# sus0pid/hsig-picotls

Measured on AMD Instinct MI355X. Metric: GiB/s AES-128-GCM seal+open, device-resident, 16KiB records, 1/2/4/8 GPU, higher is better.
Workload: dtype u8; 1 GPU; AES-128-GCM, 1M x 16 KiB TLS records, single key, per GPU (BASELINE configs[1]); records_per_gpu=1048576, record_bytes=16384, aad_bytes=5, keys=1, key_bits=128, lanes_per_record=4, record_align=128, parallelism=records sharded by range over 1 GPU(s), no collective

## Files before the change

hsig-picotls_amd/csrc/batch_kernel.h:

```cpp
#ifndef PTLS_HIP_BATCH_KERNEL_H
#define PTLS_HIP_BATCH_KERNEL_H

#include <hip/hip_runtime.h>
#include <type_traits>
#include "internal.h"

namespace ptls_hip {

constexpr uint32_t LDS_GMAIN = 0;
constexpr uint32_t LDS_AES = 65536;
constexpr uint32_t LDS_GTREE = 131072;
constexpr uint32_t LDS_TREE_STRIDE = 8192;
constexpr int TREE_TABLES = 3;
__host__ __device__ constexpr uint32_t lds_bytes(int log2g)
{
    return (void)log2g, LDS_GTREE + TREE_TABLES * LDS_TREE_STRIDE;
}

constexpr int SETPRIO = 1;
constexpr int PURE_BLOCKS = 2;
#ifndef DEAL_MUTANT
#define DEAL_MUTANT 0
#endif
#ifndef KS_STAMPS
#define KS_STAMPS 0
#endif
constexpr int QRING = 32;
constexpr uint32_t Q_END = 0xffffffffu;

struct V4 {
    uint32_t w0, w1, w2, w3;
};

__device__ __forceinline__ V4 v4xor(V4 a, V4 b)
{
    return V4{a.w0 ^ b.w0, a.w1 ^ b.w1, a.w2 ^ b.w2, a.w3 ^ b.w3};
}

__device__ __forceinline__ uint32_t xor3(uint32_t a, uint32_t b, uint32_t c)
{
    return __builtin_amdgcn_bitop3_b32(a, b, c, 0x96);
}

__device__ __forceinline__ V4 v4xor3(V4 a, V4 b, V4 c)
{
    return V4{xor3(a.w0, b.w0, c.w0), xor3(a.w1, b.w1, c.w1), xor3(a.w2, b.w2, c.w2), xor3(a.w3, b.w3, c.w3)};
}

__device__ __forceinline__ uint32_t bswap32(uint32_t x)
{
    return __builtin_bswap32(x);
}

__device__ __forceinline__ uint32_t lds32(const uint8_t *lds, uint32_t addr)
{
    return *reinterpret_cast<const uint32_t *>(lds + addr);
}

__device__ __forceinline__ V4 lds128(const uint8_t *lds, uint32_t addr)
{
    const uint4 v = *reinterpret_cast<const uint4 *>(lds + addr);
    return V4{v.x, v.y, v.z, v.w};
}

__device__ __forceinline__ void lds128_store(uint8_t *lds, uint32_t addr, V4 v)
{
    *reinterpret_cast<uint4 *>(lds + addr) = make_uint4(v.w0, v.w1, v.w2, v.w3);
}


template <int K>
__device__ __forceinline__ uint32_t aes_addr(uint32_t x, uint32_t lb)
{
    static_assert(LDS_AES == 65536, "the table base is injected as byte 2 of the address");
    return __builtin_amdgcn_perm(x, lb, 0x0c020000u | ((4u + K) << 8));
}

__device__ __forceinline__ uint32_t rotl8(uint32_t x)
{
    return __builtin_amdgcn_alignbit(x, x, 24);
}

__device__ __forceinline__ uint32_t aes_col(const uint8_t *lds, uint32_t lb, uint32_t x0, uint32_t x1, uint32_t x2, uint32_t x3,
                                            uint32_t k)
{
    const uint32_t a0 = lds32(lds, aes_addr<0>(x0, lb));
    const uint32_t a1 = lds32(lds, aes_addr<1>(x1, lb));
    const uint32_t a2 = lds32(lds, 128 + aes_addr<2>(x2, lb));
    const uint32_t a3 = lds32(lds, 128 + aes_addr<3>(x3, lb));
    return xor3(a0, a2, rotl8(a1 ^ a3)) ^ k;
}

__device__ __forceinline__ uint32_t aes_col_last(const uint8_t *lds, uint32_t lb, uint32_t x0, uint32_t x1, uint32_t x2,
                                                 uint32_t x3, uint32_t k)
{
    const uint32_t u0 = lds32(lds, 128 + aes_addr<0>(x0, lb));
    const uint32_t u1 = lds32(lds, aes_addr<1>(x1, lb));
    const uint32_t u2 = lds32(lds, aes_addr<2>(x2, lb));
    const uint32_t u3 = lds32(lds, 128 + aes_addr<3>(x3, lb));
    const uint32_t lo = __builtin_amdgcn_perm(u1, u0, 0x0c0c0500u);
    const uint32_t hi = __builtin_amdgcn_perm(u3, u2, 0x07020c0cu);
    return xor3(lo, hi, k);
}

template <int ROUNDS>
__device__ __forceinline__ V4 aes_encrypt(const uint8_t *lds, uint32_t lb, const uint32_t *__restrict__ rk, V4 s)
{
    s.w0 ^= rk[0];
    s.w1 ^= rk[1];
    s.w2 ^= rk[2];
    s.w3 ^= rk[3];
#pragma unroll
    for (int r = 1; r < ROUNDS; ++r) {
        const uint32_t t0 = aes_col(lds, lb, s.w0, s.w1, s.w2, s.w3, rk[4 * r + 0]);
        const uint32_t t1 = aes_col(lds, lb, s.w1, s.w2, s.w3, s.w0, rk[4 * r + 1]);
        const uint32_t t2 = aes_col(lds, lb, s.w2, s.w3, s.w0, s.w1, rk[4 * r + 2]);
        const uint32_t t3 = aes_col(lds, lb, s.w3, s.w0, s.w1, s.w2, rk[4 * r + 3]);
        s = V4{t0, t1, t2, t3};
    }
    const uint32_t t0 = aes_col_last(lds, lb, s.w0, s.w1, s.w2, s.w3, rk[4 * ROUNDS + 0]);
    const uint32_t t1 = aes_col_last(lds, lb, s.w1, s.w2, s.w3, s.w0, rk[4 * ROUNDS + 1]);
    const uint32_t t2 = aes_col_last(lds, lb, s.w2, s.w3, s.w0, s.w1, rk[4 * ROUNDS + 2]);
    const uint32_t t3 = aes_col_last(lds, lb, s.w3, s.w0, s.w1, s.w2, rk[4 * ROUNDS + 3]);
    return V4{t0, t1, t2, t3};
}

template <int K>
__device__ __forceinline__ uint32_t lT0(const uint8_t *lds, uint32_t x, uint32_t lb)
{
    return lds32(lds, aes_addr<K>(x, lb));
}
template <int K>
__device__ __forceinline__ uint32_t lT2(const uint8_t *lds, uint32_t x, uint32_t lb)
{
    return lds32(lds, 128 + aes_addr<K>(x, lb));
}

struct CtrConst {
    uint32_t k10, k11;
    uint32_t k20, k21, k22, k23;
    uint32_t r03;
};

__device__ __forceinline__ CtrConst ctr_const(const uint8_t *lds, uint32_t lb, const uint32_t *__restrict__ rk, uint32_t n0,
                                              uint32_t n1, uint32_t n2)
{
    const uint32_t s0 = n0 ^ rk[0], s1 = n1 ^ rk[1], s2 = n2 ^ rk[2], s3 = rk[3];
    CtrConst c;
    c.r03 = rk[3];
    c.k10 = lT0<0>(lds, s0, lb) ^ rotl8(lT0<1>(lds, s1, lb)) ^ lT2<2>(lds, s2, lb) ^ rk[4];
    c.k11 = lT0<0>(lds, s1, lb) ^ rotl8(lT0<1>(lds, s2, lb)) ^ rotl8(lT2<3>(lds, s0, lb)) ^ rk[5];
    const uint32_t t2 = lT0<0>(lds, s2, lb) ^ rotl8(lT0<1>(lds, s3, lb)) ^ lT2<2>(lds, s0, lb) ^ rotl8(lT2<3>(lds, s1, lb)) ^ rk[6];
    const uint32_t t3 = lT0<0>(lds, s3, lb) ^ rotl8(lT0<1>(lds, s0, lb)) ^ lT2<2>(lds, s1, lb) ^ rotl8(lT2<3>(lds, s2, lb)) ^ rk[7];
    c.k20 = lT2<2>(lds, t2, lb) ^ rotl8(lT2<3>(lds, t3, lb)) ^ rk[8];
    c.k21 = rotl8(lT0<1>(lds, t2, lb)) ^ lT2<2>(lds, t3, lb) ^ rk[9];
    c.k22 = lT0<0>(lds, t2, lb) ^ rotl8(lT0<1>(lds, t3, lb)) ^ rk[10];
    c.k23 = lT0<0>(lds, t3, lb) ^ rotl8(lT2<3>(lds, t2, lb)) ^ rk[11];
    return c;
}

struct RoundLoads {
    uint32_t L[16];
};

__device__ __forceinline__ void round_issue(const uint8_t *lds, uint32_t lb, const V4 &s, RoundLoads &r)
{
    const uint32_t w[4] = {s.w0, s.w1, s.w2, s.w3};
#pragma unroll
    for (int c = 0; c < 4; ++c) {
        r.L[4 * c + 0] = lds32(lds, aes_addr<0>(w[c], lb));
        r.L[4 * c + 1] = lds32(lds, aes_addr<1>(w[(c + 1) & 3], lb));
        r.L[4 * c + 2] = lds32(lds, 128 + aes_addr<2>(w[(c + 2) & 3], lb));
        r.L[4 * c + 3] = lds32(lds, 128 + aes_addr<3>(w[(c + 3) & 3], lb));
    }
}

__device__ __forceinline__ V4 round_finish(const RoundLoads &r, const uint32_t *__restrict__ k)
{
    uint32_t t[4];
#pragma unroll
    for (int c = 0; c < 4; ++c)
        t[c] = xor3(r.L[4 * c + 0], r.L[4 * c + 2], rotl8(r.L[4 * c + 1] ^ r.L[4 * c + 3])) ^ k[c];
    return V4{t[0], t[1], t[2], t[3]};
}

__device__ __forceinline__ void last_issue(const uint8_t *lds, uint32_t lb, const V4 &s, RoundLoads &r)
{
    const uint32_t w[4] = {s.w0, s.w1, s.w2, s.w3};
#pragma unroll
    for (int c = 0; c < 4; ++c) {
        r.L[4 * c + 0] = lds32(lds, 128 + aes_addr<0>(w[c], lb));
        r.L[4 * c + 1] = lds32(lds, aes_addr<1>(w[(c + 1) & 3], lb));
        r.L[4 * c + 2] = lds32(lds, aes_addr<2>(w[(c + 2) & 3], lb));
        r.L[4 * c + 3] = lds32(lds, 128 + aes_addr<3>(w[(c + 3) & 3], lb));
    }
}

__device__ __forceinline__ V4 last_finish(const RoundLoads &r, const uint32_t *__restrict__ k)
{
    uint32_t t[4];
#pragma unroll
    for (int c = 0; c < 4; ++c) {
        const uint32_t lo = __builtin_amdgcn_perm(r.L[4 * c + 1], r.L[4 * c + 0], 0x0c0c0500u);
        const uint32_t hi = __builtin_amdgcn_perm(r.L[4 * c + 3], r.L[4 * c + 2], 0x07020c0cu);
        t[c] = xor3(lo, hi, k[c]);
    }
    return V4{t[0], t[1], t[2], t[3]};
}

template <int ROUNDS, int KP, bool HASH, class GH>
__device__ __forceinline__ void ctr_ghash_skewed(const uint8_t *lds, uint32_t lb, const uint32_t *__restrict__ rk, const CtrConst &cc,
                                                 const uint32_t (&cw)[KP], V4 (&ks)[KP], V4 &y, const V4 (&hx)[KP], const GH &gm)
{
    constexpr int P = GH::PARTS;
    static_assert(P * KP <= KP * ROUNDS, "GHASH parts must fit in the segments");
    V4 s[KP];
    uint32_t t0[KP], t1[KP];
    RoundLoads R[KP];
    uint32_t M[KP][8];
    V4 G[4];
    V4 acc = V4{0, 0, 0, 0}, xr = V4{0, 0, 0, 0};
    constexpr int NSEG = KP * ROUNDS + KP - 1;
#pragma unroll
    for (int seg = 0; seg < NSEG; ++seg) {
        const int gj = seg / P, gq = seg % P;
        const bool gh = HASH && gj < KP;
        __builtin_amdgcn_s_setprio(SETPRIO);
        if (gh) {
            if (gq == 0) {
                xr = gm.prep(y);
                acc = hx[gj];
            }
            switch (gq) {
            case 0: gm.template issue<0>(lds, xr, G); break;
            case 1: gm.template issue<1>(lds, xr, G); break;
            case 2: gm.template issue<2>(lds, xr, G); break;
            case 3: gm.template issue<3 % P>(lds, xr, G); break;
            case 4: gm.template issue<4 % P>(lds, xr, G); break;
            case 5: gm.template issue<5 % P>(lds, xr, G); break;
            case 6: gm.template issue<6 % P>(lds, xr, G); break;
            default: gm.template issue<7 % P>(lds, xr, G); break;
            }
        }
        __builtin_amdgcn_sched_barrier(0);
        if (seg < KP * ROUNDS) {
            const int b = seg % KP, r = seg / KP + 1;
            if (r == 1) {
                const uint32_t x3 = cw[b] ^ cc.r03;
                M[b][0] = lT2<3>(lds, x3, lb);
                M[b][1] = lT2<2>(lds, x3, lb);
            } else if (r == 2) {
                M[b][0] = lT0<0>(lds, t0[b], lb);
                M[b][1] = lT0<1>(lds, t1[b], lb);
                M[b][2] = lT0<0>(lds, t1[b], lb);
                M[b][3] = lT2<3>(lds, t0[b], lb);
                M[b][4] = lT2<2>(lds, t0[b], lb);
                M[b][5] = lT2<3>(lds, t1[b], lb);
                M[b][6] = lT0<1>(lds, t0[b], lb);
                M[b][7] = lT2<2>(lds, t1[b], lb);
            } else if (r < ROUNDS) {
                round_issue(lds, lb, s[b], R[b]);
            } else {
                last_issue(lds, lb, s[b], R[b]);
            }
        }
        __builtin_amdgcn_sched_barrier(0);
        __builtin_amdgcn_s_setprio(0);
        if (seg >= KP - 1) {
            const int fs = seg - (KP - 1);
            const int b = fs % KP, r = fs / KP + 1;
            if (r == 1) {
                t0[b] = cc.k10 ^ rotl8(M[b][0]);
                t1[b] = cc.k11 ^ M[b][1];
            } else if (r == 2) {
                s[b].w0 = xor3(cc.k20, M[b][0], rotl8(M[b][1]));
                s[b].w1 = xor3(cc.k21, M[b][2], rotl8(M[b][3]));
                s[b].w2 = xor3(cc.k22, M[b][4], rotl8(M[b][5]));
                s[b].w3 = xor3(cc.k23, rotl8(M[b][6]), M[b][7]);
            } else if (r < ROUNDS) {
                s[b] = round_finish(R[b], rk + 4 * r);
            } else {
                ks[b] = last_finish(R[b], rk + 4 * r);
            }
        }
        if (gh) {
            acc = v4xor3(acc, G[0], G[1]);
            acc = v4xor3(acc, G[2], G[3]);
            if (gq == P - 1)
                y = acc;
        }
        __builtin_amdgcn_sched_barrier(0);
    }
}

template <int ROUNDS, int K>
__device__ __forceinline__ void aes_encrypt_n(const uint8_t *lds, uint32_t lb, const uint32_t *__restrict__ rk, V4 (&s)[K])
{
#pragma unroll
    for (int b = 0; b < K; ++b) {
        s[b].w0 ^= rk[0];
        s[b].w1 ^= rk[1];
        s[b].w2 ^= rk[2];
        s[b].w3 ^= rk[3];
    }
#pragma unroll
    for (int r = 1; r < ROUNDS; ++r) {
        const uint32_t k0 = rk[4 * r + 0], k1 = rk[4 * r + 1], k2 = rk[4 * r + 2], k3 = rk[4 * r + 3];
        V4 t[K];
#pragma unroll
        for (int b = 0; b < K; ++b) {
            t[b].w0 = aes_col(lds, lb, s[b].w0, s[b].w1, s[b].w2, s[b].w3, k0);
            t[b].w1 = aes_col(lds, lb, s[b].w1, s[b].w2, s[b].w3, s[b].w0, k1);
            t[b].w2 = aes_col(lds, lb, s[b].w2, s[b].w3, s[b].w0, s[b].w1, k2);
            t[b].w3 = aes_col(lds, lb, s[b].w3, s[b].w0, s[b].w1, s[b].w2, k3);
        }
#pragma unroll
        for (int b = 0; b < K; ++b)
            s[b] = t[b];
    }
    const uint32_t k0 = rk[4 * ROUNDS + 0], k1 = rk[4 * ROUNDS + 1], k2 = rk[4 * ROUNDS + 2], k3 = rk[4 * ROUNDS + 3];
    V4 t[K];
#pragma unroll
    for (int b = 0; b < K; ++b) {
        t[b].w0 = aes_col_last(lds, lb, s[b].w0, s[b].w1, s[b].w2, s[b].w3, k0);
        t[b].w1 = aes_col_last(lds, lb, s[b].w1, s[b].w2, s[b].w3, s[b].w0, k1);
        t[b].w2 = aes_col_last(lds, lb, s[b].w2, s[b].w3, s[b].w0, s[b].w1, k2);
        t[b].w3 = aes_col_last(lds, lb, s[b].w3, s[b].w0, s[b].w1, s[b].w2, k3);
    }
#pragma unroll
    for (int b = 0; b < K; ++b)
        s[b] = t[b];
}


struct GhLane {
    uint32_t lb0, lb1, lb2, lb3;
    uint32_t shift;
    bool rot1, rot2;
};

__device__ __forceinline__ GhLane gh_lane_from(uint32_t lane)
{
    GhLane g;
    const uint32_t base = lane * 0x01010101u + 0x03020100u;
    g.lb0 = ((base + 0x00000000u) & 0x0f0f0f0fu) << 4;
    g.lb1 = ((base + 0x04040404u) & 0x0f0f0f0fu) << 4;
    g.lb2 = ((base + 0x08080808u) & 0x0f0f0f0fu) << 4;
    g.lb3 = ((base + 0x0c0c0c0cu) & 0x0f0f0f0fu) << 4;
    g.shift = 8u * (lane & 3);
    g.rot1 = ((lane >> 2) & 1) != 0;
    g.rot2 = ((lane >> 3) & 1) != 0;
    return g;
}

__device__ __forceinline__ GhLane gh_lane_init(int lane)
{
    return gh_lane_from((uint32_t)lane);
}

template <int K>
__device__ __forceinline__ V4 gh_term(const uint8_t *lds, uint32_t xw, uint32_t lbw)
{
    const uint32_t addr = __builtin_amdgcn_perm(xw, lbw, 0x0c0c0000u | ((4u + (K & 3)) << 8) | (K & 3));
    return lds128(lds, LDS_GMAIN + addr);
}

__device__ __forceinline__ V4 gh_mul_main(const uint8_t *lds, const GhLane &g, V4 y, V4 x)
{
    const uint32_t s0 = g.rot1 ? y.w1 : y.w0, s1 = g.rot1 ? y.w2 : y.w1, s2 = g.rot1 ? y.w3 : y.w2, s3 = g.rot1 ? y.w0 : y.w3;
    const uint32_t r0 = g.rot2 ? s2 : s0, r1 = g.rot2 ? s3 : s1, r2 = g.rot2 ? s0 : s2, r3 = g.rot2 ? s1 : s3;
    const uint32_t x0 = __builtin_amdgcn_alignbit(r1, r0, g.shift);
    const uint32_t x1 = __builtin_amdgcn_alignbit(r2, r1, g.shift);
    const uint32_t x2 = __builtin_amdgcn_alignbit(r3, r2, g.shift);
    const uint32_t x3 = __builtin_amdgcn_alignbit(r0, r3, g.shift);
    V4 acc = v4xor3(x, gh_term<0>(lds, x0, g.lb0), gh_term<1>(lds, x0, g.lb0));
    acc = v4xor3(acc, gh_term<2>(lds, x0, g.lb0), gh_term<3>(lds, x0, g.lb0));
    acc = v4xor3(acc, gh_term<4>(lds, x1, g.lb1), gh_term<5>(lds, x1, g.lb1));
    acc = v4xor3(acc, gh_term<6>(lds, x1, g.lb1), gh_term<7>(lds, x1, g.lb1));
    acc = v4xor3(acc, gh_term<8>(lds, x2, g.lb2), gh_term<9>(lds, x2, g.lb2));
    acc = v4xor3(acc, gh_term<10>(lds, x2, g.lb2), gh_term<11>(lds, x2, g.lb2));
    acc = v4xor3(acc, gh_term<12>(lds, x3, g.lb3), gh_term<13>(lds, x3, g.lb3));
    acc = v4xor3(acc, gh_term<14>(lds, x3, g.lb3), gh_term<15>(lds, x3, g.lb3));
    return acc;
}

__device__ __forceinline__ V4 gh_rot(const GhLane &g, V4 y)
{
    const uint32_t s0 = g.rot1 ? y.w1 : y.w0, s1 = g.rot1 ? y.w2 : y.w1, s2 = g.rot1 ? y.w3 : y.w2, s3 = g.rot1 ? y.w0 : y.w3;
    const uint32_t r0 = g.rot2 ? s2 : s0, r1 = g.rot2 ? s3 : s1, r2 = g.rot2 ? s0 : s2, r3 = g.rot2 ? s1 : s3;
    return V4{__builtin_amdgcn_alignbit(r1, r0, g.shift), __builtin_amdgcn_alignbit(r2, r1, g.shift),
              __builtin_amdgcn_alignbit(r3, r2, g.shift), __builtin_amdgcn_alignbit(r0, r3, g.shift)};
}

template <int T0, int NT, int NG>
__device__ __forceinline__ void gh_issue(const uint8_t *lds, const GhLane &g, const V4 &xr, V4 (&G)[NG])
{
    static_assert(NT <= NG, "lookups must fit the result array");
#pragma unroll
    for (int i = 0; i < NT; ++i) {
        const int t = T0 + i, q = t >> 2;
        const uint32_t xw = q == 0 ? xr.w0 : q == 1 ? xr.w1 : q == 2 ? xr.w2 : xr.w3;
        const uint32_t lbw = q == 0 ? g.lb0 : q == 1 ? g.lb1 : q == 2 ? g.lb2 : g.lb3;
        const uint32_t addr = __builtin_amdgcn_perm(xw, lbw, 0x0c0c0000u | ((4u + (t & 3)) << 8) | (t & 3));
        G[i] = lds128(lds, LDS_GMAIN + addr);
    }
}

struct GhMain {
    const GhLane &g;
    static constexpr int PARTS = 4;
    __device__ __forceinline__ V4 prep(V4 y) const { return gh_rot(g, y); }
    template <int Q>
    __device__ __forceinline__ void issue(const uint8_t *lds, const V4 &xr, V4 (&G)[4]) const
    {
        gh_issue<4 * Q, 4>(lds, g, xr, G);
    }
};

struct GhNibble {
    uint32_t tab;
    static constexpr int PARTS = 8;
    __device__ __forceinline__ V4 prep(V4 y) const { return y; }
    template <int Q>
    __device__ __forceinline__ void issue(const uint8_t *lds, const V4 &xr, V4 (&G)[4]) const
    {
        const uint32_t w = (Q >> 1) == 0 ? xr.w0 : (Q >> 1) == 1 ? xr.w1 : (Q >> 1) == 2 ? xr.w2 : xr.w3;
#pragma unroll
        for (int i = 0; i < 4; ++i) {
            const int j = 4 * (Q & 1) + i;
            G[i] = lds128(lds, tab + (uint32_t)(8 * (Q >> 1) + j) * 256u + ((w >> (4 * j)) & 15u) * 16u);
        }
    }
};

template <int ROUNDS, int KP, bool HASH>
__device__ __forceinline__ void ctr_ghash(const uint8_t *lds, uint32_t lb, const uint32_t *__restrict__ rk, const CtrConst &cc,
                                          const uint32_t (&cw)[KP], V4 (&ks)[KP], V4 &y, const V4 (&hx)[KP], const GhLane &g)
{
    ctr_ghash_skewed<ROUNDS, KP, HASH>(lds, lb, rk, cc, cw, ks, y, hx, GhMain{g});
}

__device__ __forceinline__ V4 gh_mul_nibble(const uint8_t *lds, uint32_t table, V4 y)
{
    V4 acc = V4{0, 0, 0, 0};
    const uint32_t w[4] = {y.w0, y.w1, y.w2, y.w3};
#pragma unroll
    for (int i = 0; i < 4; ++i) {
        V4 t[8];
#pragma unroll
        for (int j = 0; j < 8; ++j)
            t[j] = lds128(lds, table + (uint32_t)(8 * i + j) * 256u + ((w[i] >> (4 * j)) & 15u) * 16u);
        acc = v4xor3(acc, t[0], t[1]);
        acc = v4xor3(acc, t[2], t[3]);
        acc = v4xor3(acc, t[4], t[5]);
        acc = v4xor3(acc, t[6], t[7]);
        __builtin_amdgcn_sched_barrier(0);
    }
    return acc;
}

__device__ __forceinline__ void mulx_be(uint32_t (&v)[4])
{
    const uint32_t c = (uint32_t)__builtin_amdgcn_sbfe((int)v[3], 0u, 1u);
    v[3] = __builtin_amdgcn_alignbit(v[2], v[3], 1);
    v[2] = __builtin_amdgcn_alignbit(v[1], v[2], 1);
    v[1] = __builtin_amdgcn_alignbit(v[0], v[1], 1);
    v[0] = (v[0] >> 1) ^ (c & 0xe1000000u);
}

template <int NT, int STRIDE = 1024>
struct Win4 {
    uint32_t base;
    uint32_t y[4];
};

template <int NT>
__device__ __forceinline__ Win4<NT> gf_win4_build(uint8_t *lds, uint32_t tab, int lane, V4 yr)
{
    static_assert(NT == 8 || NT == 16, "4-bit windows: 8 or 16 table entries per lane");
    uint32_t m[4][4];
    m[0][0] = bswap32(yr.w0), m[0][1] = bswap32(yr.w1), m[0][2] = bswap32(yr.w2), m[0][3] = bswap32(yr.w3);
#pragma unroll
    for (int k = 1; k < 4; ++k) {
#pragma unroll
        for (int w = 0; w < 4; ++w)
            m[k][w] = m[k - 1][w];
        mulx_be(m[k]);
    }
    Win4<NT> t;
    uint32_t zero;
    asm volatile("v_mov_b32 %0, 0" : "=v"(zero));
    uint32_t ln = (uint32_t)lane;
    asm volatile("" : "+v"(ln));
    t.base = tab + ln * 16u;
#pragma unroll
    for (int w = 0; w < 4; ++w)
        t.y[w] = m[0][w];
#pragma unroll
    for (int n = 0; n < NT; ++n) {
        uint32_t e[4] = {zero, zero, zero, zero};
#pragma unroll
        for (int k = 0; k < 4; ++k)
            if ((n >> (3 - k)) & 1)
#pragma unroll
                for (int w = 0; w < 4; ++w)
                    e[w] ^= m[k][w];
        lds128_store(lds, t.base + (uint32_t)n * 1024u, V4{e[0], e[1], e[2], e[3]});
    }
    return t;
}

template <int NT, int LB = 8, int STRIDE>
__device__ __forceinline__ V4 gf_win4_mul(const uint8_t *lds, const Win4<NT, STRIDE> &tb, V4 xr)
{
    static_assert(LB == 8 || LB == 4 || LB == 2, "lookups in flight: 8, 4 or 2");
    const uint32_t x[4] = {bswap32(xr.w0), bswap32(xr.w1), bswap32(xr.w2), bswap32(xr.w3)};
    uint32_t z0 = 0, z1 = 0, z2 = 0, z3 = 0, ov = 0;
#pragma unroll
    for (int g = 0; g < 32 / LB; ++g) {
        const int j0 = 31 - g * LB, w = j0 >> 3, i0 = 8 * w + 7 - j0;
        V4 t[LB];
#pragma unroll
// ... 466 lines not shown
                    if (__hip_atomic_fetch_add(queue + 1, 1u, __ATOMIC_RELAXED, __HIP_MEMORY_SCOPE_AGENT) == gridDim.x - 1) {
                        __hip_atomic_store(queue, 0u, __ATOMIC_RELAXED, __HIP_MEMORY_SCOPE_AGENT);
                        __hip_atomic_store(queue + 1, 0u, __ATOMIC_RELAXED, __HIP_MEMORY_SCOPE_AGENT);
                    }
                }
                __hip_atomic_store(ent, (uint64_t)k << 32 | c, __ATOMIC_RELAXED, __HIP_MEMORY_SCOPE_WORKGROUP);
            } else {
                uint64_t v;
                while (((v = __hip_atomic_load(ent, __ATOMIC_RELAXED, __HIP_MEMORY_SCOPE_WORKGROUP)) >> 32) != k)
                    __builtin_amdgcn_s_sleep(2);
                c = (uint32_t)v;
            }
        }
        return __builtin_amdgcn_readfirstlane(c);
    };
    const uint32_t lb_aes = (uint32_t)(lane & 31) * 4u | LDS_AES;
    const GhLane gl = gh_lane_init(lane);
    const int r = lane & (G - 1);
    const int grp = lane >> LOG2G;

    clock_stamp(clk, 0);
    build_aes_tables<WGT>(lds, LDS_AES, t0);
    uint64_t ks_acc[16] = {};
    const uint64_t ks_t0 = KS_STAMPS ? __builtin_amdgcn_s_memtime() : 0;
    uint64_t ks_last = ks_t0;
    auto ks_phase = [&](int k) __attribute__((always_inline)) {
        if (KS_STAMPS) {
            const uint64_t t = __builtin_amdgcn_s_memtime();
            ks_acc[k] += t - ks_last;
            ks_last = t;
        }
    };
    uint32_t cur_key = 0xffffffffu;
    uint32_t g = 0, cbase = 0;
    bool have_g = false;

    for (uint32_t ci = use_q ? next_chunk() : blockIdx.x; ci < nchunks; ci = use_q ? next_chunk() : ci + gridDim.x) {
        const Chunk ch = chunks[ci];
        if (ch.key != cur_key) {
            const uint64_t s0 = KS_STAMPS ? __builtin_amdgcn_s_memtime() : 0;
            __syncthreads();
            const uint64_t s1 = KS_STAMPS ? __builtin_amdgcn_s_memtime() : 0;
            build_ghash_tables(lds, basis + (size_t)ch.key * (BASIS_VECS * 4), LOG2G);
            if (threadIdx.x == 0 && (DEAL_MUTANT != 3 || cur_key == 0xffffffffu))
                *task_ctr = 0;
            if (KS_STAMPS)
                __builtin_amdgcn_s_waitcnt(0);
            const uint64_t s2 = KS_STAMPS ? __builtin_amdgcn_s_memtime() : 0;
            __syncthreads();
            if (KS_STAMPS) {
                const uint64_t s3 = __builtin_amdgcn_s_memtime();
                ks_acc[1] += s1 - s0;
                ks_acc[2] += s2 - s1;
                ks_acc[3] += s3 - s2;
                ks_acc[4] += 1;
                ks_last = s3;
            }
            cur_key = ch.key;
            cbase = 0;
            have_g = false;
        }
        if (DEAL_MUTANT == 1)
            have_g = false;

        const KeySlot *__restrict__ slot = slots + ch.key;
        const uint32_t *__restrict__ rk = slot->rk;
        const int ntasks = (int)((ch.count + R - 1) / R);

        for (;;) {
            if (!have_g) {
                uint32_t v = 0;
                if (lane == 0)
                    v = __hip_atomic_fetch_add(task_ctr, 1u, __ATOMIC_RELAXED, __HIP_MEMORY_SCOPE_WORKGROUP);
                g = __builtin_amdgcn_readfirstlane(v);
                have_g = true;
            }
            const int t = (int)(g - cbase);
            if (t >= ntasks)
                break;
            have_g = false;
            ks_phase(5);
            const uint32_t ridx = (uint32_t)t * R + grp;
            const bool valid = ridx < ch.count;
            const uint32_t pos = ch.first + (valid ? ridx : 0);
            const ptls_hip_record_t rec = recs_ord[pos];
            const uint32_t rec_i = order != nullptr ? order[pos] : pos;
            const int L = valid ? (int)rec.len : 0;
            const int A = valid ? (int)rec.aad_len : 0;
            const int na = (A + 15) >> 4, nc = (L + 15) >> 4;
            const int N = valid ? na + nc + 1 : 0;
            const int i0 = (r + na) & (G - 1);
            const int my_iters = N > i0 ? ((N - 1 - i0) >> LOG2G) + 1 : 0;

            const bool tflag = !OPEN && (rec.flags & 1u) != 0 && L > 0;
            const uint32_t ttype = (rec.flags >> 8) & 0xffu;
            const uint8_t *in_p = in + rec.in_off;
            uint8_t *out_p = out + rec.out_off;
            const uint8_t *aad_p = aad + rec.aad_off;
            const uint32_t n0 = slot->iv[0], n1 = slot->iv[1] ^ bswap32((uint32_t)(rec.seq >> 32)),
                           n2 = slot->iv[2] ^ bswap32((uint32_t)rec.seq);

            V4 y = V4{0, 0, 0, 0}, ek0 = V4{0, 0, 0, 0};
            CtrConst cc;

            auto generic_pair = [&](int m) {
                Elem e[2];
                V4 in[2], ks[2];
                uint32_t cw[2];
                int big = 0;
                int sft[2];
#pragma unroll
                for (int b = 0; b < 2; ++b) {
                    e[b] = elem_of(i0 + (m + b) * G, N, na, nc, L, N);
                    in[b] = V4{0, 0, 0, 0};
                    sft[b] = 0;
                    if (e[b].is_c) {
                        const bool tb = tflag && e[b].c == nc - 1;
                        in[b] = tail_load(in_p + 16 * (size_t)e[b].c, e[b].c, e[b].nbytes - (tb ? 1 : 0), sft[b]);
                    }
                    cw[b] = e[b].is_c ? bswap32((uint32_t)e[b].c + 2u) : 0x01000000u;
                    ks[b] = V4{n0, n1, n2, cw[b]};
                    big |= (e[b].is_c && e[b].c >= 65534) ? 1 : 0;
                }
                const int bigw = wave_max(big);
                ks_phase(10);
                if (bigw != 0) {
                    aes_encrypt_n<ROUNDS, 2>(lds, lb_aes, rk, ks);
                } else {
                    const V4 nohash[2] = {V4{0, 0, 0, 0}, V4{0, 0, 0, 0}};
                    V4 ydummy = V4{0, 0, 0, 0};
                    ctr_ghash<ROUNDS, 2, false>(lds, lb_aes, rk, cc, cw, ks, ydummy, nohash, gl);
                }
                if (KS_STAMPS)
                    __builtin_amdgcn_s_waitcnt(0xc07f);
                ks_phase(11);
                V4 xs[2];
#pragma unroll
                for (int b = 0; b < 2; ++b) {
                    in[b] = tail_shift(in[b], sft[b]);
                    if (tflag && e[b].is_c && e[b].c == nc - 1)
                        in[b] = put_byte(in[b], e[b].nbytes - 1, ttype);
                    xs[b] = finish_elem<OPEN, ALIGNED>(e[b], in[b], ks[b], aad_p, A, L, out_p, ek0);
                }
                if (KS_STAMPS)
                    __builtin_amdgcn_s_waitcnt(0);
                ks_phase(12);
#pragma unroll
                for (int b = 0; b < 2; ++b)
                    if (e[b].active)
                        y = gh_mul_main(lds, gl, y, xs[b]);
                if (KS_STAMPS)
                    __builtin_amdgcn_s_waitcnt(0);
                ks_phase(13);
            };

            auto generic_iter_m = [&](int m) {
                const Elem e0 = elem_of(i0 + m * G, N, na, nc, L, N);
                V4 in0 = V4{0, 0, 0, 0};
                int sft0 = 0;
                const bool tb0 = tflag && e0.is_c && e0.c == nc - 1;
                if (e0.is_c)
                    in0 = tail_load(in_p + 16 * (size_t)e0.c, e0.c, e0.nbytes - (tb0 ? 1 : 0), sft0);
                const uint32_t cw0[1] = {e0.is_c ? bswap32((uint32_t)e0.c + 2u) : 0x01000000u};
                V4 ks0[1] = {V4{n0, n1, n2, cw0[0]}};
                if (wave_max((e0.is_c && e0.c >= 65534) ? 1 : 0) == 0) {
                    const V4 nohash[1] = {V4{0, 0, 0, 0}};
                    V4 ydummy = V4{0, 0, 0, 0};
                    ctr_ghash<ROUNDS, 1, false>(lds, lb_aes, rk, cc, cw0, ks0, ydummy, nohash, gl);
                } else {
                    aes_encrypt_n<ROUNDS, 1>(lds, lb_aes, rk, ks0);
                }
                in0 = tail_shift(in0, sft0);
                if (tb0)
                    in0 = put_byte(in0, e0.nbytes - 1, ttype);
                const V4 x0 = finish_elem<OPEN, ALIGNED>(e0, in0, ks0[0], aad_p, A, L, out_p, ek0);
                if (e0.active)
                    y = gh_mul_main(lds, gl, y, x0);
            };

            constexpr int KP = PURE_BLOCKS;
            const int nf = (L - (tflag ? 1 : 0)) >> 4;
            const int pm0 = na > i0 ? (na - i0 + G - 1) >> LOG2G : 0;
            const int lastc = min(nf, 65534) - 1;
            const int my_mhi = min((valid && na + lastc - i0 >= 0) ? ((na + lastc - i0) >> LOG2G) + 1 : 0, my_iters);
            const int npure = -wave_max(-max(my_mhi - pm0, 0)) / KP;
            const int pm1 = pm0 + npure * KP;

            const int naad = wave_max(pm0);
            for (int j = 0; j < naad; ++j) {
                if (j < pm0) {
                    const int ia = i0 + j * G;
                    const V4 x = ALIGNED ? load_block_nb(aad_p + 16 * ia, min(16, A - 16 * ia), reinterpret_cast<const uint8_t *>(t0))
                                         : load_block<false>(aad_p + 16 * ia, min(16, A - 16 * ia));
                    y = j == 0 ? x : gh_mul_main(lds, gl, y, x);
                }
            }
            cc = ctr_const(lds, lb_aes, rk, n0, n1, n2);
            ks_phase(6);
            if (npure) {
                const uint8_t *src = in_p + 16 * (size_t)(i0 - na + pm0 * G);
                uint8_t *dst = out_p + 16 * (size_t)(i0 - na + pm0 * G);
                const uint32_t cbase = (uint32_t)(i0 - na + pm0 * G) + 2u;
                V4 pend[KP], bufA[KP], bufB[KP];
                constexpr bool DEFER_OK = !OPEN && ALIGNED && KP * G >= 8;
                bool spill[KP];
                int defer_any = 0;
                {
                    const int lo = DEFER_OK ? (int)(((uint32_t)(uintptr_t)out_p >> 4) & 7u) : 0;
                    const int jr = (i0 - na) & (G - 1);
#pragma unroll
                    for (int b = 0; b < KP; ++b) {
                        spill[b] = DEFER_OK && lo != 0 && jr + b * G >= KP * G - lo;
                        defer_any |= spill[b] ? 1 : 0;
                    }
                }
#pragma unroll
                for (int b = 0; b < KP; ++b)
                    bufA[b] = load_full(src + 16 * b * G);
                auto put = [&](auto defer_tag, int it, bool first, int b, const V4 &c, const V4 &held) __attribute__((always_inline)) {
                    constexpr bool DEFER = decltype(defer_tag)::value;
                    const size_t o = (size_t)(it * KP * G) * 16;
                    if (!DEFER) {
                        store_full(dst + o + 16 * b * G, c);
                    } else if (first) {
                        if (!spill[b])
                            store_full(dst + o + 16 * b * G, c);
                    } else {
                        const size_t op = (size_t)((it - 1) * KP * G) * 16;
                        store_full(dst + (spill[b] ? op : o) + 16 * b * G, spill[b] ? held : c);
                    }
                };
                auto stretch = [&](auto defer_tag) __attribute__((always_inline)) {
                    constexpr bool DEFER = decltype(defer_tag)::value;
                    auto pure_iter = [&](int it, bool hash_pending, V4(&d)[KP], V4(&dn)[KP]) __attribute__((always_inline)) {
                        const size_t on = (size_t)(min(it + 1, npure - 1) * KP * G) * 16;
                        V4 k[KP];
                        uint32_t cw[KP];
#pragma unroll
                        for (int b = 0; b < KP; ++b) {
                            dn[b] = load_full(src + on + 16 * b * G);
                            cw[b] = bswap32(cbase + (uint32_t)((it * KP + b) * G));
                            k[b] = V4{n0, n1, n2, cw[b]};
                        }
                        __builtin_amdgcn_sched_barrier(0);
                        if (OPEN) {
                            ctr_ghash<ROUNDS, KP, true>(lds, lb_aes, rk, cc, cw, k, y, d, gl);
#pragma unroll
                            for (int b = 0; b < KP; ++b) {
                                store_full(dst + (size_t)(it * KP * G) * 16 + 16 * b * G, v4xor(d[b], k[b]));
                            }
                        } else {
                            if (hash_pending)
                                ctr_ghash<ROUNDS, KP, true>(lds, lb_aes, rk, cc, cw, k, y, pend, gl);
                            else
                                ctr_ghash<ROUNDS, KP, false>(lds, lb_aes, rk, cc, cw, k, y, pend, gl);
#pragma unroll
                            for (int b = 0; b < KP; ++b) {
                                const V4 c = v4xor(d[b], k[b]);
                                put(defer_tag, it, !hash_pending, b, c, pend[b]);
                                pend[b] = c;
                            }
                        }
                    };
                    pure_iter(0, false, bufA, bufB);
                    int it = 1;
                    for (; it + 1 < npure; it += 2) {
                        pure_iter(it, true, bufB, bufA);
                        pure_iter(it + 1, true, bufA, bufB);
                    }
                    if (it < npure)
                        pure_iter(it, true, bufB, bufA);
                    if (DEFER) {
#pragma unroll
                        for (int b = 0; b < KP; ++b)
                            if (spill[b])
                                store_full(dst + (size_t)((npure - 1) * KP * G) * 16 + 16 * b * G, pend[b]);
                    }
                };
                if (DEFER_OK && wave_max(defer_any) != 0)
                    stretch(std::true_type{});
                else
                    stretch(std::false_type{});
                if (!OPEN) {
#pragma unroll
                    for (int b = 0; b < KP; ++b)
                        y = gh_mul_main(lds, gl, y, pend[b]);
                }
            }
            ks_phase(7);
            {
                const int rest = wave_max(max(my_iters - pm1, 0));
                int j = 0;
                for (; j + 1 < rest; j += 2)
                    generic_pair(pm1 + j);
                if (j < rest)
                    generic_iter_m(pm1 + j);
            }

            ks_phase(8);
            const int q = (N - 1 - na - r) & (G - 1);
            V4 s;
            if constexpr (G >= 2) {
                constexpr int WCP = win_copies(G);
                Win4<16, 16 * win_row(G)> wt;
                wt.base = LDS_GTREE + (uint32_t)(q * WCP + (grp & (WCP - 1))) * 16u;
                s = group_xor<G>(gf_win4_mul<16, 4>(lds, wt, y));
            }
            if (valid && q == 0) {
                if constexpr (G == 1)
                    s = gh_mul_nibble(lds, LDS_GTREE, y);
                const V4 tag = v4xor(s, ek0);
                if (OPEN) {
                    const V4 rt = load_full(in_p + L);
                    const bool ok = rt.w0 == tag.w0 && rt.w1 == tag.w1 && rt.w2 == tag.w2 && rt.w3 == tag.w3;
                    result[rec_i] = ok ? (uint64_t)L : ~(uint64_t)0;
                } else {
                    store_full(out_p + L, tag);
                }
            }
            if (!OPEN && supp != nullptr) {
                __builtin_amdgcn_fence(__ATOMIC_RELEASE, "workgroup");
                __builtin_amdgcn_fence(__ATOMIC_ACQUIRE, "workgroup");
                if (valid && r == 0) {
                    const ptls_hip_supp_t sp = supp[rec_i];
                    if ((sp.flags & PTLS_HIP_SUPP_ENABLE) && sp.hp_key < hp_nslots) {
                        const V4 sample = load_full(out + sp.sample_off);
                        const V4 m = aes_encrypt<ROUNDS>(lds, lb_aes, hp_slots[sp.hp_key].rk, sample);
                        store_full(mask + sp.mask_off, m);
                    }
                }
            }
            ks_phase(9);
        }
        if (DEAL_MUTANT != 2)
            cbase += (uint32_t)ntasks;
    }
    if (KS_STAMPS && clk != nullptr) {
        ks_acc[0] = __builtin_amdgcn_s_memtime() - ks_t0;
        uint64_t *o = clk + 4 * (size_t)gridDim.x + 16 * ((size_t)blockIdx.x * NW + (size_t)wave);
#pragma unroll
        for (int k = 0; k < 16; ++k)
            if (lane == k)
                o[k] = ks_acc[k];
    }
    if (clk != nullptr) {
        __syncthreads();
        clock_stamp(clk, 1);
    }
}

template <int G, int R, bool O, int W>
static hipError_t launch_one(unsigned grid, hipStream_t s, const KernelArgs &a, bool aligned)
{
    if (KS_STAMPS && a.clk != nullptr && a.clk_bytes < 8 * (4 * (size_t)grid + 16 * (size_t)grid * (W / 64)))
        return hipErrorInvalidValue;
    if (aligned)
        hipLaunchKernelGGL((aesgcm_batch_kernel<G, R, O, true, W>), dim3(grid), dim3(W), 0, s, a.recs_ord, a.order, a.chunks,
                           a.nchunks, a.in, a.aad, a.out, a.result, a.slots, a.basis, a.t0, a.supp, a.hp_slots, a.hp_nslots, a.mask, a.clk,
                           a.queue);
    else
        hipLaunchKernelGGL((aesgcm_batch_kernel<G, R, O, false, W>), dim3(grid), dim3(W), 0, s, a.recs_ord, a.order, a.chunks,
                           a.nchunks, a.in, a.aad, a.out, a.result, a.slots, a.basis, a.t0, a.supp, a.hp_slots, a.hp_nslots, a.mask, a.clk,
                           a.queue);
    return hipGetLastError();
}
// ... 22 lines not shown
```

Baseline: 1242 GiB/s.

## Cache counter-window partial state to cut AES round 1-2 table lookups in CTR

Adds a per-block counter window (CtrWin) that precomputes the part of AES round 2 that depends only on counter byte 1. Within a 256-counter window, rounds 1 and 2 then need only 5 LDS table lookups instead of 10. The window is updated incrementally (wave-uniform ballot) when counters cross a window boundary, and this path is used for lane groups G<=4. In exchange it holds extra registers for the window state, runs a step on each crossing, and reloads the record and recomputes the counter constants after the stretch, which raises register pressure.

```diff
diff --git a/hsig-picotls_amd/csrc/batch_kernel.h b/hsig-picotls_amd/csrc/batch_kernel.h
--- a/hsig-picotls_amd/csrc/batch_kernel.h
+++ b/hsig-picotls_amd/csrc/batch_kernel.h
@@ -4,6 +4,7 @@
 #include <hip/hip_runtime.h>
 #include <type_traits>
 #include "internal.h"
+#include "ctr_window.h"
 
 namespace ptls_hip {
 
@@ -136,28 +137,28 @@
     return lds32(lds, 128 + aes_addr<K>(x, lb));
 }
 
-struct CtrConst {
-    uint32_t k10, k11;
-    uint32_t k20, k21, k22, k23;
-    uint32_t r03;
+struct LdsTab {
+    const uint8_t *lds;
+    uint32_t lb;
+    template <int K>
+    __device__ __forceinline__ uint32_t t0(uint32_t x) const { return lT0<K>(lds, x, lb); }
+    template <int K>
+    __device__ __forceinline__ uint32_t t2(uint32_t x) const { return lT2<K>(lds, x, lb); }
 };
 
 __device__ __forceinline__ CtrConst ctr_const(const uint8_t *lds, uint32_t lb, const uint32_t *__restrict__ rk, uint32_t n0,
                                               uint32_t n1, uint32_t n2)
 {
-    const uint32_t s0 = n0 ^ rk[0], s1 = n1 ^ rk[1], s2 = n2 ^ rk[2], s3 = rk[3];
-    CtrConst c;
-    c.r03 = rk[3];
-    c.k10 = lT0<0>(lds, s0, lb) ^ rotl8(lT0<1>(lds, s1, lb)) ^ lT2<2>(lds, s2, lb) ^ rk[4];
-    c.k11 = lT0<0>(lds, s1, lb) ^ rotl8(lT0<1>(lds, s2, lb)) ^ rotl8(lT2<3>(lds, s0, lb)) ^ rk[5];
-    const uint32_t t2 = lT0<0>(lds, s2, lb) ^ rotl8(lT0<1>(lds, s3, lb)) ^ lT2<2>(lds, s0, lb) ^ rotl8(lT2<3>(lds, s1, lb)) ^ rk[6];
-    const uint32_t t3 = lT0<0>(lds, s3, lb) ^ rotl8(lT0<1>(lds, s0, lb)) ^ lT2<2>(lds, s1, lb) ^ rotl8(lT2<3>(lds, s2, lb)) ^ rk[7];
-    c.k20 = lT2<2>(lds, t2, lb) ^ rotl8(lT2<3>(lds, t3, lb)) ^ rk[8];
-    c.k21 = rotl8(lT0<1>(lds, t2, lb)) ^ lT2<2>(lds, t3, lb) ^ rk[9];
-    c.k22 = lT0<0>(lds, t2, lb) ^ rotl8(lT0<1>(lds, t3, lb)) ^ rk[10];
-    c.k23 = lT0<0>(lds, t3, lb) ^ rotl8(lT2<3>(lds, t2, lb)) ^ rk[11];
-    return c;
-}
+    return ctr_const(LdsTab{lds, lb}, rk, n0, n1, n2);
+}
+
+__host__ __device__ constexpr bool ctr_window_form(int g)
+{
+    return g <= 4;
+}
+
+struct NoWin {
+};
 
 struct RoundLoads {
     uint32_t L[16];
@@ -208,16 +209,20 @@
     return V4{t[0], t[1], t[2], t[3]};
 }
 
-template <int ROUNDS, int KP, bool HASH, class GH>
+template <int ROUNDS, int KP, bool HASH, class GH, class WN>
 __device__ __forceinline__ void ctr_ghash_skewed(const uint8_t *lds, uint32_t lb, const uint32_t *__restrict__ rk, const CtrConst &cc,
-                                                 const uint32_t (&cw)[KP], V4 (&ks)[KP], V4 &y, const V4 (&hx)[KP], const GH &gm)
+                                                 const uint32_t (&cw)[KP], V4 (&ks)[KP], V4 &y, const V4 (&hx)[KP], const GH &gm,
+                                                 const WN &wn)
 {
     constexpr int P = GH::PARTS;
+    constexpr bool WIN = !std::is_same<WN, NoWin>::value;
     static_assert(P * KP <= KP * ROUNDS, "GHASH parts must fit in the segments");
+    const LdsTab tab{lds, lb};
     V4 s[KP];
     uint32_t t0[KP], t1[KP];
     RoundLoads R[KP];
     uint32_t M[KP][8];
+    uint32_t MW[KP][4];
     V4 G[4];
     V4 acc = V4{0, 0, 0, 0}, xr = V4{0, 0, 0, 0};
     constexpr int NSEG = KP * ROUNDS + KP - 1;
@@ -245,7 +250,14 @@
         __builtin_amdgcn_sched_barrier(0);
         if (seg < KP * ROUNDS) {
             const int b = seg % KP, r = seg / KP + 1;
-            if (r == 1) {
+            if (WIN && r <= 2) {
+                if constexpr (WIN) {
+                    if (r == 1)
+                        MW[b][0] = ctrw_r1_issue(tab, cc, cw[b]);
+                    else
+                        ctrw_r2_issue(tab, t0[b], MW[b]);
+                }
+            } else if (r == 1) {
                 const uint32_t x3 = cw[b] ^ cc.r03;
                 M[b][0] = lT2<3>(lds, x3, lb);
                 M[b][1] = lT2<2>(lds, x3, lb);
@@ -269,7 +281,17 @@
         if (seg >= KP - 1) {
             const int fs = seg - (KP - 1);
             const int b = fs % KP, r = fs / KP + 1;
-            if (r == 1) {
+            if (WIN && r <= 2) {
+                if constexpr (WIN) {
+                    if (r == 1) {
+                        t0[b] = ctrw_r1_finish(cc, MW[b][0]);
+                    } else {
+                        uint32_t c[4];
+                        ctrw_r2_finish(wn[b], MW[b], c);
+                        s[b] = V4{c[0], c[1], c[2], c[3]};
+                    }
+                }
+            } else if (r == 1) {
                 t0[b] = cc.k10 ^ rotl8(M[b][0]);
                 t1[b] = cc.k11 ^ M[b][1];
             } else if (r == 2) {
@@ -291,6 +313,13 @@
         }
         __builtin_amdgcn_sched_barrier(0);
     }
+}
+
+template <int ROUNDS, int KP, bool HASH, class GH>
+__device__ __forceinline__ void ctr_ghash_skewed(const uint8_t *lds, uint32_t lb, const uint32_t *__restrict__ rk, const CtrConst &cc,
+                                                 const uint32_t (&cw)[KP], V4 (&ks)[KP], V4 &y, const V4 (&hx)[KP], const GH &gm)
+{
+    ctr_ghash_skewed<ROUNDS, KP, HASH>(lds, lb, rk, cc, cw, ks, y, hx, gm, NoWin{});
 }
 
 template <int ROUNDS, int K>
@@ -438,6 +467,17 @@
                                           const uint32_t (&cw)[KP], V4 (&ks)[KP], V4 &y, const V4 (&hx)[KP], const GhLane &g)
 {
     ctr_ghash_skewed<ROUNDS, KP, HASH>(lds, lb, rk, cc, cw, ks, y, hx, GhMain{g});
+}
+
+template <int ROUNDS, int KP, bool HASH, bool WIN>
+__device__ __forceinline__ void ctr_ghash_stretch(const uint8_t *lds, uint32_t lb, const uint32_t *__restrict__ rk, const CtrConst &cc,
+                                                  const CtrWin (&wn)[KP], const uint32_t (&cw)[KP], V4 (&ks)[KP], V4 &y,
+                                                  const V4 (&hx)[KP], const GhLane &g)
+{
+    if constexpr (WIN)
+        ctr_ghash_skewed<ROUNDS, KP, HASH>(lds, lb, rk, cc, cw, ks, y, hx, GhMain{g}, wn);
+    else
+        ctr_ghash_skewed<ROUNDS, KP, HASH>(lds, lb, rk, cc, cw, ks, y, hx, GhMain{g}, NoWin{});
 }
 
 __device__ __forceinline__ V4 gh_mul_nibble(const uint8_t *lds, uint32_t table, V4 y)
@@ -1070,23 +1110,28 @@
             ks_phase(5);
             const uint32_t ridx = (uint32_t)t * R + grp;
             const bool valid = ridx < ch.count;
-            const uint32_t pos = ch.first + (valid ? ridx : 0);
-            const ptls_hip_record_t rec = recs_ord[pos];
-            const uint32_t rec_i = order != nullptr ? order[pos] : pos;
-            const int L = valid ? (int)rec.len : 0;
-            const int A = valid ? (int)rec.aad_len : 0;
-            const int na = (A + 15) >> 4, nc = (L + 15) >> 4;
-            const int N = valid ? na + nc + 1 : 0;
-            const int i0 = (r + na) & (G - 1);
-            const int my_iters = N > i0 ? ((N - 1 - i0) >> LOG2G) + 1 : 0;
-
-            const bool tflag = !OPEN && (rec.flags & 1u) != 0 && L > 0;
-            const uint32_t ttype = (rec.flags >> 8) & 0xffu;
-            const uint8_t *in_p = in + rec.in_off;
-            uint8_t *out_p = out + rec.out_off;
-            const uint8_t *aad_p = aad + rec.aad_off;
-            const uint32_t n0 = slot->iv[0], n1 = slot->iv[1] ^ bswap32((uint32_t)(rec.seq >> 32)),
-                           n2 = slot->iv[2] ^ bswap32((uint32_t)rec.seq);
+            uint32_t rec_i, ttype, n0, n1, n2;
+            int L, A, na, nc, N, i0, my_iters;
+            bool tflag;
+            const uint8_t *in_p, *aad_p;
+            uint8_t *out_p;
+            auto load_rec = [&](uint32_t pos) __attribute__((always_inline)) {
+                const ptls_hip_record_t rec = recs_ord[pos];
+                rec_i = order != nullptr ? order[pos] : pos;
+                L = valid ? (int)rec.len : 0;
+                A = valid ? (int)rec.aad_len : 0;
+                na = (A + 15) >> 4, nc = (L + 15) >> 4;
+                N = valid ? na + nc + 1 : 0;
+                i0 = (r + na) & (G - 1);
+                my_iters = N > i0 ? ((N - 1 - i0) >> LOG2G) + 1 : 0;
+                tflag = !OPEN && (rec.flags & 1u) != 0 && L > 0;
+                ttype = (rec.flags >> 8) & 0xffu;
+                in_p = in + rec.in_off;
+                out_p = out + rec.out_off;
+                aad_p = aad + rec.aad_off;
+                n0 = slot->iv[0], n1 = slot->iv[1] ^ bswap32((uint32_t)(rec.seq >> 32)), n2 = slot->iv[2] ^ bswap32((uint32_t)rec.seq);
+            };
+            load_rec(ch.first + (valid ? ridx : 0));
 
             V4 y = V4{0, 0, 0, 0}, ek0 = V4{0, 0, 0, 0};
             CtrConst cc;
@@ -1190,6 +1235,8 @@
                 uint8_t *dst = out_p + 16 * (size_t)(i0 - na + pm0 * G);
                 const uint32_t cbase = (uint32_t)(i0 - na + pm0 * G) + 2u;
                 V4 pend[KP], bufA[KP], bufB[KP];
+                constexpr bool WINF = ctr_window_form(G);
+                CtrWin wn[KP];
                 constexpr bool DEFER_OK = !OPEN && ALIGNED && KP * G >= 8;
                 bool spill[KP];
                 int defer_any = 0;
@@ -1218,6 +1265,21 @@
                         store_full(dst + (spill[b] ? op : o) + 16 * b * G, spill[b] ? held : c);
                     }
                 };
+                auto win_refresh = [&](int itn) __attribute__((always_inline)) {
+                    if constexpr (WINF) {
+                        const LdsTab tab{lds, lb_aes};
+                        bool cross = false;
+#pragma unroll
+                        for (int b = 0; b < KP; ++b)
+                            cross |= ctr_window_crossed(cbase + (uint32_t)((itn * KP + b) * G), (uint32_t)(KP * G));
+                        if (__builtin_amdgcn_ballot_w64(cross) != 0) {
+#pragma unroll
+                            for (int b = 0; b < KP; ++b)
+                                wn[b] = ctr_window_step(tab, cc.k11, cc.r03, wn[b], bswap32(cbase + (uint32_t)(((itn - 1) * KP + b) * G)),
+                                                        bswap32(cbase + (uint32_t)((itn * KP + b) * G)));
+                        }
+                    }
+                };
                 auto stretch = [&](auto defer_tag) __attribute__((always_inline)) {
                     constexpr bool DEFER = decltype(defer_tag)::value;
                     auto pure_iter = [&](int it, bool hash_pending, V4(&d)[KP], V4(&dn)[KP]) __attribute__((always_inline)) {
@@ -1231,17 +1293,19 @@
                             k[b] = V4{n0, n1, n2, cw[b]};
                         }
                         __builtin_amdgcn_sched_barrier(0);
+                        if (it != 0)
+                            win_refresh(it);
                         if (OPEN) {
-                            ctr_ghash<ROUNDS, KP, true>(lds, lb_aes, rk, cc, cw, k, y, d, gl);
+                            ctr_ghash_stretch<ROUNDS, KP, true, WINF>(lds, lb_aes, rk, cc, wn, cw, k, y, d, gl);
 #pragma unroll
                             for (int b = 0; b < KP; ++b) {
                                 store_full(dst + (size_t)(it * KP * G) * 16 + 16 * b * G, v4xor(d[b], k[b]));
                             }
                         } else {
                             if (hash_pending)
-                                ctr_ghash<ROUNDS, KP, true>(lds, lb_aes, rk, cc, cw, k, y, pend, gl);
+                                ctr_ghash_stretch<ROUNDS, KP, true, WINF>(lds, lb_aes, rk, cc, wn, cw, k, y, pend, gl);
                             else
-                                ctr_ghash<ROUNDS, KP, false>(lds, lb_aes, rk, cc, cw, k, y, pend, gl);
+                                ctr_ghash_stretch<ROUNDS, KP, false, WINF>(lds, lb_aes, rk, cc, wn, cw, k, y, pend, gl);
 #pragma unroll
                             for (int b = 0; b < KP; ++b) {
                                 const V4 c = v4xor(d[b], k[b]);
@@ -1265,10 +1329,21 @@
                                 store_full(dst + (size_t)((npure - 1) * KP * G) * 16 + 16 * b * G, pend[b]);
                     }
                 };
+                if constexpr (WINF) {
+#pragma unroll
+                    for (int b = 0; b < KP; ++b)
+                        wn[b] = ctr_window(LdsTab{lds, lb_aes}, cc, bswap32(cbase + (uint32_t)(b * G)));
+                }
                 if (DEFER_OK && wave_max(defer_any) != 0)
                     stretch(std::true_type{});
                 else
                     stretch(std::false_type{});
+                if constexpr (WINF) {
+                    uint32_t pos = ch.first + (valid ? ridx : 0);
+                    asm volatile("" : "+v"(pos));
+                    load_rec(pos);
+                    cc = ctr_const(lds, lb_aes, rk, n0, n1, n2);
+                }
                 if (!OPEN) {
 #pragma unroll
                     for (int b = 0; b < KP; ++b)
diff --git a/hsig-picotls_amd/csrc/ctr_window.h b/hsig-picotls_amd/csrc/ctr_window.h
--- /dev/null
+++ b/hsig-picotls_amd/csrc/ctr_window.h
@@ -0,0 +1,138 @@
+#pragma once
+
+#include <stdint.h>
+
+#ifndef GF128_FN
+#define GF128_FN __host__ __device__ __forceinline__
+#endif
+#define CTRW_FN GF128_FN
+
+namespace ptls_hip {
+
+CTRW_FN uint32_t ctrw_rotl8(uint32_t x)
+{
+    return (x << 8) | (x >> 24);
+}
+
+struct CtrConst {
+    uint32_t k10, k11;
+    uint32_t k20, k21, k22, k23;
+    uint32_t r03;
+};
+
+struct CtrWin {
+    uint32_t w0, w1, w2, w3;
+};
+
+template <class TAB>
+CTRW_FN CtrConst ctr_const(const TAB &tab, const uint32_t *rk, uint32_t n0, uint32_t n1, uint32_t n2)
+{
+    const uint32_t s0 = n0 ^ rk[0], s1 = n1 ^ rk[1], s2 = n2 ^ rk[2], s3 = rk[3];
+    CtrConst c;
+    c.r03 = rk[3];
+    c.k10 = tab.template t0<0>(s0) ^ ctrw_rotl8(tab.template t0<1>(s1)) ^ tab.template t2<2>(s2) ^ rk[4];
+    c.k11 = tab.template t0<0>(s1) ^ ctrw_rotl8(tab.template t0<1>(s2)) ^ ctrw_rotl8(tab.template t2<3>(s0)) ^ rk[5];
+    const uint32_t t2 = tab.template t0<0>(s2) ^ ctrw_rotl8(tab.template t0<1>(s3)) ^ tab.template t2<2>(s0) ^
+                        ctrw_rotl8(tab.template t2<3>(s1)) ^ rk[6];
+    const uint32_t t3 = tab.template t0<0>(s3) ^ ctrw_rotl8(tab.template t0<1>(s0)) ^ tab.template t2<2>(s1) ^
+                        ctrw_rotl8(tab.template t2<3>(s2)) ^ rk[7];
+    c.k20 = tab.template t2<2>(t2) ^ ctrw_rotl8(tab.template t2<3>(t3)) ^ rk[8];
+    c.k21 = ctrw_rotl8(tab.template t0<1>(t2)) ^ tab.template t2<2>(t3) ^ rk[9];
+    c.k22 = tab.template t0<0>(t2) ^ ctrw_rotl8(tab.template t0<1>(t3)) ^ rk[10];
+    c.k23 = tab.template t0<0>(t3) ^ ctrw_rotl8(tab.template t2<3>(t2)) ^ rk[11];
+    return c;
+}
+
+CTRW_FN uint32_t ctr_window_of(uint32_t ctr)
+{
+    return ctr >> 8;
+}
+
+CTRW_FN bool ctr_window_crossed(uint32_t ctr, uint32_t step)
+{
+    return (ctr & 255u) < step;
+}
+
+template <class TAB>
+CTRW_FN uint32_t ctr_window_t1(const TAB &tab, uint32_t k11, uint32_t r03, uint32_t cw)
+{
+    return k11 ^ tab.template t2<2>(cw ^ r03);
+}
+
+template <int W, class TAB>
+CTRW_FN uint32_t ctr_window_term(const TAB &tab, uint32_t t1)
+{
+    static_assert(W >= 0 && W < 4, "state column");
+    return W == 0 ? ctrw_rotl8(tab.template t0<1>(t1))
+         : W == 1 ? tab.template t0<0>(t1)
+         : W == 2 ? ctrw_rotl8(tab.template t2<3>(t1))
+                  : tab.template t2<2>(t1);
+}
+
+template <class TAB>
+CTRW_FN CtrWin ctr_window(const TAB &tab, const CtrConst &c, uint32_t cw)
+{
+    const uint32_t t1 = ctr_window_t1(tab, c.k11, c.r03, cw);
+    CtrWin w;
+    w.w0 = c.k20 ^ ctr_window_term<0>(tab, t1);
+    w.w1 = c.k21 ^ ctr_window_term<1>(tab, t1);
+    w.w2 = c.k22 ^ ctr_window_term<2>(tab, t1);
+    w.w3 = c.k23 ^ ctr_window_term<3>(tab, t1);
+    return w;
+}
+
+template <int W, class TAB>
+CTRW_FN uint32_t ctr_window_step_col(const TAB &tab, uint32_t w, uint32_t t1o, uint32_t t1n)
+{
+    return w ^ ctr_window_term<W>(tab, t1o) ^ ctr_window_term<W>(tab, t1n);
+}
+
+template <class TAB>
+CTRW_FN CtrWin ctr_window_step(const TAB &tab, uint32_t k11, uint32_t r03, const CtrWin &w, uint32_t cwo, uint32_t cwn)
+{
+    const uint32_t to = ctr_window_t1(tab, k11, r03, cwo), tn = ctr_window_t1(tab, k11, r03, cwn);
+    CtrWin n;
+    n.w0 = ctr_window_step_col<0>(tab, w.w0, to, tn);
+    n.w1 = ctr_window_step_col<1>(tab, w.w1, to, tn);
+    n.w2 = ctr_window_step_col<2>(tab, w.w2, to, tn);
+    n.w3 = ctr_window_step_col<3>(tab, w.w3, to, tn);
+    return n;
+}
+
+template <class TAB>
+CTRW_FN uint32_t ctrw_r1_issue(const TAB &tab, const CtrConst &c, uint32_t cw)
+{
+    return tab.template t2<3>(cw ^ c.r03);
+}
+
+CTRW_FN uint32_t ctrw_r1_finish(const CtrConst &c, uint32_t m)
+{
+    return c.k10 ^ ctrw_rotl8(m);
+}
+
+template <class TAB>
+CTRW_FN void ctrw_r2_issue(const TAB &tab, uint32_t t0, uint32_t (&m)[4])
+{
+    m[0] = tab.template t0<0>(t0);
+    m[1] = tab.template t2<3>(t0);
+    m[2] = tab.template t2<2>(t0);
+    m[3] = tab.template t0<1>(t0);
+}
+
+CTRW_FN void ctrw_r2_finish(const CtrWin &w, const uint32_t (&m)[4], uint32_t (&s)[4])
+{
+    s[0] = w.w0 ^ m[0];
+    s[1] = w.w1 ^ ctrw_rotl8(m[1]);
+    s[2] = w.w2 ^ m[2];
+    s[3] = w.w3 ^ ctrw_rotl8(m[3]);
+}
+
+template <class TAB>
+CTRW_FN void ctr_rounds12_window(const TAB &tab, const CtrConst &c, const CtrWin &w, uint32_t cw, uint32_t (&s)[4])
+{
+    uint32_t m[4];
+    ctrw_r2_issue(tab, ctrw_r1_finish(c, ctrw_r1_issue(tab, c, cw)), m);
+    ctrw_r2_finish(w, m, s);
+}
+
+}
```

New measurement: 1259 GiB/s (median of 6 runs). 1.4% higher.
